# XuyangBai/D3Feat

Measured on AMD Instinct MI355X. Metric: fragments/sec (30k-pt clouds), higher is better.
Workload: dtype f32; 1 GPU; SURVEY §8d config #2: synthetic 3DMatch room fragment, 300k raw pts -> grid subsample 0.03 m (~29k pts per cloud) -> self-pair -> 5-level pyramid -> full KPFCNN forward (random-init weights (reference initialiser, seed 42), 14.1M params)...; points_per_cloud=29369, fragments_per_gpu=2141, parallelism=fragment-dp1, fragments_per_replay=12, engine_fallbacks=0, engine_isolated_replays=0

## Files before the change

### d3feat_amd/_lib.py

```python
import ctypes as C
import os

_HERE = os.path.dirname(os.path.abspath(__file__))
LIB_PATH = os.environ.get("D3FEAT_AMD_LIB") or os.path.join(_HERE, "lib", "libd3feat_amd.so")

D3F_OK = 0
ERRORS = {-1: "HIP runtime / kernel launch failure", -2: "workspace too small", -3: "invalid argument"}
ST_EMPTY_ELEMENT, ST_NEG_CELL, ST_KEY_RANGE, ST_HIT_OVERFLOW, ST_OUT_OVERFLOW, ST_KEY_WIDTH = 1, 2, 4, 8, 16, 32
PAD_NUM_SUPPORTS = -2147483648
NEIGHBOR_CAP = 1024
MAX_BATCH = 255
TOPK_MAX = 8192
PAIRS_KMAX = 1024

_vp, _sz, _i, _f = C.c_void_p, C.c_size_t, C.c_int, C.c_float

SIGNATURES = {
    "d3f_version": (_i, []),
    "d3f_trace_marker": (_i, [_i, _vp]),
    "d3f_pack_status": (_i, [_vp, _vp, _i, _vp, _i, _vp, _i, _vp, _i, _vp, _i, _i, _i, _vp]),
    "d3f_grid_subsample_workspace_bytes": (_sz, [_i, _i, _i, _i]),
    "d3f_batch_grid_subsample": (_i, [_vp, _i, _vp, _i, _f, _vp, _i, _vp, _i, _vp, _vp, _vp, _vp, _vp, _vp, _sz, _vp]),
    "d3f_batch_grid_subsample_async": (_i, [_vp, _i, _vp, _i, _f, _vp, _i, _i, _i, _vp, _vp, _vp, _sz, _vp]),
    "d3f_batch_grid_subsample_async_inplace": (_i, [_vp, _i, _vp, _i, _f, _vp, _i, _i, _vp, _vp, _vp, _sz, _vp]),
    "d3f_stack_self_pair": (_i, [_vp, _i, _vp, _i, _vp, _vp, _vp, _vp]),
    "d3f_radius_neighbors_workspace_bytes": (_sz, [_i, _i, _i]),
    "d3f_batch_radius_neighbors": (_i, [_vp, _i, _vp, _i, _vp, _vp, _i, _f, _vp, _i, _i, _i, _vp, _vp, _sz, _vp]),
    "d3f_neighbor_grid_bytes": (_sz, [_i, _i]),
    "d3f_neighbor_grid_order_offset": (_sz, [_i, _i]),
    "d3f_neighbor_grid_build": (_i, [_vp, _i, _vp, _i, _f, _vp, _sz, _vp]),
    "d3f_neighbor_grid_search": (_i, [_vp, _sz, _i, _vp, _i, _vp, _i, _f, _i, _vp, _i, _i, _i, _i, _i, _f, _i, _vp, _vp]),
    "d3f_neighbor_grid_search_ordered": (_i, [_vp, _sz, _i, _vp, _i, _vp, _i, _f, _vp, _sz, _vp, _i, _i, _i, _i, _i, _f, _i, _vp, _vp]),
    "d3f_neighbor_grid_inv_offset": (_sz, [_i, _i]),
    "d3f_neighbor_grid_xyz_offset": (_sz, [_i, _i]),
    "d3f_row_positive": (_i, [_vp, _i, _i, _i, _vp, _vp, _i, _vp]),
    "d3f_kpconv_aggregate": (_i, [_vp, _i, _vp, _i, _vp, _i, _i, _vp, _i, _i, _vp, _vp, _i, _f, _i, _i, _vp, _vp, _vp, _vp,
                                  _vp, _i, _vp]),
    "d3f_kpconv_fused_c1": (_i, [_vp, _i, _vp, _i, _vp, _i, _i, _vp, _i, _vp, _i, _f, _i, _i, _vp, _i, _vp, _vp, _vp, _i, _i,
                                 _f, _vp, _i, _vp, _vp, _vp, _i, _vp]),
    "d3f_kpconv_fused32": (_i, [_vp, _i, _vp, _i, _vp, _i, _i, _vp, _i, _vp, _vp, _i, _f, _i, _i, _vp, _vp, _vp, _vp, _i, _i, _f, _vp,
                                _i, _vp, _vp, _vp, _i, _vp]),
    "d3f_kpconv_fused_supported": (_i, [_i, _i, _i, _i, _i]),
    "d3f_kpconv_pack_weights": (_i, [_vp, _i, _i, _vp, _vp]),
    "d3f_kpconv_fused": (_i, [_vp, _i, _vp, _i, _vp, _i, _i, _vp, _i, _i, _vp, _vp, _i, _f, _i, _i, _vp, _i, _vp, _vp, _vp, _i, _i,
                              _f, _vp, _i, _vp, _vp, _vp, _i, _vp]),
    "d3f_kpconv_fused32_x3": (_i, [_vp, _i, _vp, _i, _vp, _i, _i, _vp, _i, _vp, _vp, _i, _f, _i, _i, _vp, _vp, _vp, _vp, _i, _i, _f, _vp,
                                   _i, _vp, _vp, _vp, _i, _vp]),
    "d3f_kpconv_packed_x3_bytes": (_sz, [_i, _i]),
    "d3f_kpconv_pack_weights_x3": (_i, [_vp, _i, _i, _vp, _vp]),
    "d3f_kpconv_fused_x3": (_i, [_vp, _i, _vp, _i, _vp, _i, _i, _vp, _i, _i, _vp, _vp, _i, _f, _i, _i, _vp, _i, _vp, _vp, _vp, _i, _i,
                                 _f, _vp, _i, _vp, _vp, _vp, _i, _vp]),
    "d3f_gemm_workspace_bytes": (_sz, [_i, _i, _i, _i]),
    "d3f_gemm_bf16_workspace_bytes": (_sz, [_i, _i, _i, _i]),
    "d3f_gemm_f32": (_i, [_vp, _i, _vp, _i, _vp, _i, _i, _i, _i, _vp, _vp, _vp, _vp, _i, _i, _f, _vp, _sz, _vp, _i, _vp]),
    "d3f_gemm_upsample_cat_f32": (_i, [_vp, _i, _i, _i, _vp, _i, _vp, _i, _i, _vp, _i, _vp, _i, _i, _i, _vp, _vp, _i, _f, _vp, _sz,
                                       _vp, _vp, _i, _vp]),
    "d3f_ind_max_pool": (_i, [_vp, _i, _i, _i, _vp, _i, _i, _i, _vp, _i, _vp, _vp, _vp, _vp, _i, _vp]),
    "d3f_closest_pool_cat": (_i, [_vp, _i, _i, _i, _vp, _i, _i, _vp, _i, _i, _vp, _i, _vp, _vp, _vp]),
    "d3f_affine_act": (_i, [_vp, _i, _i, _i, _vp, _vp, _vp, _i, _i, _f, _vp, _i, _vp, _vp]),
    "d3f_pack_descriptors": (_i, [_vp, _vp, _i, _i, _vp, _i, _vp, _i, _vp, _vp]),
    "d3f_pack_descriptors_to": (_i, [_vp, _vp, _i, _i, _vp, _i, _vp, _i, _vp, _vp, _i, _i, _i, _vp, _vp, _vp]),
    "d3f_topk_workspace_bytes": (_sz, [_i, _i, _i, _i]),
    "d3f_topk_records": (_i, [_vp, _i, _vp, _i, _i, _vp, _i, _i, _vp, _vp, _i, _i, _i, _vp, _i, _i, _vp, _i, _vp, _vp, _vp, _vp, _sz,
                              _vp]),
    "d3f_feature_nn_workspace_bytes": (_sz, [_i]),
    "d3f_feature_nn": (_i, [_vp, _i, _i, _vp, _i, _i, _i, _vp, _vp, _vp, _sz, _vp]),
    "d3f_mutual_matches_workspace_bytes": (_sz, [_i]),
    "d3f_mutual_matches": (_i, [_vp, _i, _vp, _i, _vp, _vp, _vp, _sz, _vp]),
    "d3f_ransac_hypotheses": (_i, [_vp, _i, _vp, _i, _vp, _i, _f, _f, C.c_uint64, C.c_uint64, _i, _vp, _vp, _vp]),
    "d3f_ransac_draw": (_i, [C.c_uint64, C.c_uint64, _i, _i]),
    "d3f_neighbor_grid_score": (_i, [_vp, _sz, _i, _vp, _i, _vp, _i, _f, _vp, _vp, _vp, _vp]),
    "d3f_register_pairs_workspace_bytes": (_sz, [_i, _i, _i, _i]),
    "d3f_register_pairs": (_i, [_vp, _i, _i, _i, _i, _vp, _vp, _i, _i, _f, _i, _f, _f, _i, _i, C.c_uint64, _vp, _f] + [_vp] * 11
                           + [_sz, _vp]),
# ... 45 lines not shown
```

### d3feat_amd/csrc/grid_subsample.hip

```cpp
#include <cstdlib>
#include "prims.h"
#include "radix_sort.h"

#define GS_EMPTY 0xFFFFFFFFFFFFFFFFull
#define GS_KEYBITS 56
#define GS_KEYMASK ((1ull << GS_KEYBITS) - 1ull)
#define GS_MAX_PROBE 4096

__constant__ unsigned long long D3F_CHAIN_DEV[D3F_NCHAIN] = {
    13ull, 29ull, 59ull, 127ull, 257ull, 541ull, 1109ull, 2357ull, 5087ull, 10273ull, 20753ull, 42043ull, 85229ull,
    172933ull, 351061ull, 712697ull, 1447153ull, 2938679ull, 5967347ull, 12117689ull, 24607243ull, 49969847ull,
    101473717ull, 206062531ull, 418451333ull, 849749479ull, 1725587117ull, 3504151727ull};

struct GsElem {
    float org[3];
    int pad0;
    unsigned long long NX, NY, NZ;
    long long bbase;
};

static unsigned long long gs_chain_ge(long long n) {
    for (int j = 0; j < D3F_NCHAIN; ++j)
        if ((long long)D3F_CHAIN_HOST[j] >= n) return D3F_CHAIN_HOST[j];
    return D3F_CHAIN_HOST[D3F_NCHAIN - 1];
// ... 11 lines not shown
}
__device__ __forceinline__ void gs_prep(const unsigned* __restrict__ bbox, const int* __restrict__ offs, int B, float dl,
                                        GsElem* __restrict__ el, int* __restrict__ status, RsMeta* __restrict__ smeta,
                                        int n_cap) {
    __shared__ unsigned long long sCells[256];
    const int b = threadIdx.x;
    unsigned long long cells = 0ull;
    if (b < B) {
        GsElem e;
        e.pad0 = 0;
        const int len = offs[b + 1] - offs[b];
        if (len <= 0) {
            atomicOr(&status[1], D3F_ST_EMPTY_ELEMENT);
            e.org[0] = e.org[1] = e.org[2] = 0.f;
            e.NX = e.NY = e.NZ = 1;
        } else {
            const float inv = __fdiv_rn(1.0f, dl);
            float mx[3];
#pragma unroll
            for (int d = 0; d < 3; ++d) {
                float mn = d3f_ord2f(__hip_atomic_load(&bbox[b * 6 + d], __ATOMIC_RELAXED, __HIP_MEMORY_SCOPE_AGENT));
                mx[d] = d3f_ord2f(__hip_atomic_load(&bbox[b * 6 + 3 + d], __ATOMIC_RELAXED, __HIP_MEMORY_SCOPE_AGENT));
                e.org[d] = __fmul_rn(floorf(__fmul_rn(mn, inv)), dl);
            }
            e.NX = (unsigned long long)fmaxf(floorf(__fdiv_rn(__fsub_rn(mx[0], e.org[0]), dl)), 0.f) + 1ull;
            e.NY = (unsigned long long)fmaxf(floorf(__fdiv_rn(__fsub_rn(mx[1], e.org[1]), dl)), 0.f) + 1ull;
            e.NZ = (unsigned long long)fmaxf(floorf(__fdiv_rn(__fsub_rn(mx[2], e.org[2]), dl)), 0.f) + 1ull;
        }
        long long base = 0;
        for (int j = 0; j < b; ++j) {
            long long l = offs[j + 1] - offs[j];
            unsigned long long nb = D3F_CHAIN_DEV[D3F_NCHAIN - 1];
            for (int c = 0; c < D3F_NCHAIN; ++c)
                if ((long long)D3F_CHAIN_DEV[c] >= l) { nb = D3F_CHAIN_DEV[c]; break; }
            base += (long long)nb;
        }
        e.bbase = base;
        el[b] = e;
        const double c = (double)e.NX * (double)e.NY * (double)e.NZ;
        cells = c >= 1.8e19 ? 0xFFFFFFFFFFFFFFFFull : e.NX * e.NY * e.NZ;
    }
    if (!smeta) return;
    sCells[threadIdx.x] = cells;
    __syncthreads();
    if (threadIdx.x == 0) {
        unsigned long long mx = 1ull;
        for (int j = 0; j < B; ++j) mx = sCells[j] > mx ? sCells[j] : mx;
        int kb = gs_bits(mx - 1ull);
        if (kb < 1) kb = 1;
        const int eb = gs_bits((unsigned long long)(B - 1));
        RsMeta m;
        m.n = min(offs[B], n_cap);
        m.kb = kb;
        m.bits = kb + eb;
        if (m.bits > 32) {
            atomicOr(&status[1], D3F_ST_KEY_WIDTH);
            m.n = 0;
            m.bits = 8;
        }
        m.npass = (m.bits + 7) / 8;
        *smeta = m;
    }
}
struct GsPrepEpi {
    const unsigned* bbox; const int* offs; int B; float dl; GsElem* el; int* status; RsMeta* smeta; int n_cap;
    __device__ __forceinline__ void operator()() const { gs_prep(bbox, offs, B, dl, el, status, smeta, n_cap); }
};

__global__ void __launch_bounds__(256) gs_insert_kernel(const float* __restrict__ pts, int N, const int* __restrict__ offs,
                                                        int B, float dl, const GsElem* __restrict__ el,
                                                        unsigned long long* __restrict__ tkey, unsigned* __restrict__ tfirst,
                                                        unsigned long long capmask, int* __restrict__ slot,
                                                        int* __restrict__ status) {
    const int i = blockIdx.x * blockDim.x + threadIdx.x;
    if (i >= min(N, offs[B])) return;
    const int b = d3f_find_elem(offs, B, i);
    const GsElem e = el[b];
    const float fx = floorf(__fdiv_rn(__fsub_rn(pts[3 * (size_t)i + 0], e.org[0]), dl));
    const float fy = floorf(__fdiv_rn(__fsub_rn(pts[3 * (size_t)i + 1], e.org[1]), dl));
    const float fz = floorf(__fdiv_rn(__fsub_rn(pts[3 * (size_t)i + 2], e.org[2]), dl));
    int st = 0;
    if (fx < 0.f || fy < 0.f || fz < 0.f) st |= D3F_ST_NEG_CELL;
    const unsigned long long ix = (unsigned long long)fmaxf(fx, 0.f), iy = (unsigned long long)fmaxf(fy, 0.f),
                             iz = (unsigned long long)fmaxf(fz, 0.f);
    const unsigned long long key = ix + e.NX * iy + e.NX * e.NY * iz;
    if (key > GS_KEYMASK) st |= D3F_ST_KEY_RANGE;
    if (st) atomicOr(&status[1], st);
    const unsigned long long word = ((unsigned long long)b << GS_KEYBITS) | (key & GS_KEYMASK);
    unsigned long long h = gs_mix(word) & capmask;
    bool placed = false;
    for (int probe = 0; probe < GS_MAX_PROBE; ++probe) {
        unsigned long long prev = atomicCAS(&tkey[h], GS_EMPTY, word);
        if (prev == GS_EMPTY || prev == word) { placed = true; break; }
        h = (h + 1) & capmask;
    }
    if (!placed) atomicOr(&status[1], D3F_ST_OUT_OVERFLOW);
    atomicMin(&tfirst[h], (unsigned)i);
    slot[i] = (int)h;
}

struct GsMarkIn {
    const int* n_dev; const int* slot; const unsigned* tfirst;
    __device__ __forceinline__ int operator()(int i) const { return (i < *n_dev && tfirst[slot[i]] == (unsigned)i) ? 1 : 0; }
};

__global__ void __launch_bounds__(256) gs_chain_kernel(int N, const int* __restrict__ slot, const unsigned* __restrict__ tfirst,
                                                       const unsigned long long* __restrict__ tkey,
                                                       const int* __restrict__ vscan, const int* __restrict__ vbase,
                                                       int* __restrict__ pvid,
                                                       unsigned long long* __restrict__ vkey, int* __restrict__ vhead,
                                                       int* __restrict__ vcnt, int* __restrict__ pnext,
                                                       const int* __restrict__ n_dev) {
    const int i = blockIdx.x * blockDim.x + threadIdx.x;
// ... 291 lines not shown
        int run = wbase + x - s;
#pragma unroll
        for (int k = 0; k < 4; ++k) {
            const int u = tile * GS_TILE + tid * 4 + k;
            if (u < hi) A.cd[o + hi - 1 - u] = run;
            run += c[k];
        }
        if (tid == 0) A.tsum[o / GS_TILE + b + tile] = tot;
    }
    if (!d3f_last_block(counter + b, (unsigned)((hi + GS_TILE - 1) / GS_TILE))) return;
    gs_order_scan_sums(A, j, b, wsum);
}

__global__ void __launch_bounds__(256) gs_order_place_kernel(GsOrderArgs A, int j) {
    const int b = blockIdx.y;
    int M, lo, hi, nb;
    bool last;
    if (!gs_round(A, b, j, M, lo, hi, nb, last)) return;
    const int t = blockIdx.x * 256 + threadIdx.x;
    const int o = A.offs[b];
    const long long bbase = A.el[b].bbase;
    const bool next = !last && j + 1 < D3F_NCHAIN;
    const int nbn = next ? (int)D3F_CHAIN_DEV[j + 1] : 1;
    int id = -1, pos = -1;
    if (t < hi) {
        id = (t < lo) ? A.P[j & 1][o + t] : t;
        const int bk = A.bkt[j & 1][o + t];
        int r = 0;
        for (int q = A.bh[j & 1][bbase + bk]; q >= 0; q = A.nx[j & 1][o + q]) r += (q > t) ? 1 : 0;
        const int f = A.bf[j & 1][bbase + bk];
        const int dest = A.cd[o + f] + A.tsum[o / GS_TILE + b + (hi - 1 - f) / GS_TILE] + r;
        A.P[(j + 1) & 1][o + dest] = id;
        if (last) A.vpos[A.moffs[b] + id] = dest;
        pos = dest;
    } else if (next && t < min(M, nbn)) {
        id = pos = t;
    }
    if (next && id >= 0) {
        const int bk = gs_mod(A.vkey[A.moffs[b] + id], (unsigned)nbn, 1.0 / (double)nbn);
        atomicMin(&A.bf[(j + 1) & 1][bbase + bk], pos);
        atomicAdd(&A.bc[(j + 1) & 1][bbase + bk], 1);
        A.nx[(j + 1) & 1][o + pos] = atomicExch(&A.bh[(j + 1) & 1][bbase + bk], pos);
        A.bkt[(j + 1) & 1][o + pos] = bk;
    }
}

#include "gs_small.h"

__global__ void __launch_bounds__(RS_THREADS) gs_sortkey_kernel(const float* __restrict__ pts, const float* const* __restrict__ ptrs,
                                                                const int* __restrict__ offs, int B,
                                                                float dl, const GsElem* __restrict__ el,
                                                                const RsMeta* __restrict__ smeta, unsigned* __restrict__ skey,
                                                                unsigned* __restrict__ hist, int* __restrict__ status) {
    __shared__ unsigned sHist[256];
    __shared__ int sOffs[D3F_MAX_BATCH + 1];
    __shared__ GsElem sEl[D3F_MAX_BATCH];
    __shared__ const float* sBase[D3F_MAX_BATCH];
    const int n = smeta->n, kb = smeta->kb;
    const int tile = blockIdx.x;
    if ((long long)tile * RS_TILE >= (long long)n) return;
    for (int t = threadIdx.x; t <= B; t += RS_THREADS) sOffs[t] = offs[t];
    for (int t = threadIdx.x; t < B; t += RS_THREADS) {
        sEl[t] = el[t];
        sBase[t] = ptrs ? ptrs[t] - 3 * (size_t)offs[t] : pts;
    }
    __syncthreads();
    const int w = threadIdx.x >> 6, lane = threadIdx.x & 63;
    const int base = tile * RS_TILE + w * RS_WAVE_ITEMS + lane;
    const int wlo = tile * RS_TILE + w * RS_WAVE_ITEMS, whi = min(wlo + RS_WAVE_ITEMS, n) - 1;
    int b0 = 0;
    while (b0 + 1 < B && wlo >= sOffs[b0 + 1]) ++b0;
    const bool one_cloud = (b0 + 1 >= B) || whi < sOffs[b0 + 1];
    unsigned key[RS_ROUNDS], vm = 0u;
    int st = 0;
#pragma unroll
    for (int r = 0; r < RS_ROUNDS; ++r) {
        const int i = base + r * 64;
        key[r] = 0u;
        if (i < n) {
            int b = b0;
            if (!one_cloud)
                while (b + 1 < B && i >= sOffs[b + 1]) ++b;
            const float ox = sEl[b].org[0], oy = sEl[b].org[1], oz = sEl[b].org[2];
            const unsigned NX = (unsigned)sEl[b].NX, NY = (unsigned)sEl[b].NY;
            const float* __restrict__ P = sBase[b];
            const float fx = floorf(__fdiv_rn(__fsub_rn(P[3 * (size_t)i + 0], ox), dl));
            const float fy = floorf(__fdiv_rn(__fsub_rn(P[3 * (size_t)i + 1], oy), dl));
            const float fz = floorf(__fdiv_rn(__fsub_rn(P[3 * (size_t)i + 2], oz), dl));
            if (fx < 0.f || fy < 0.f || fz < 0.f) st |= D3F_ST_NEG_CELL;
            const unsigned ix = (unsigned)fmaxf(fx, 0.f), iy = (unsigned)fmaxf(fy, 0.f), iz = (unsigned)fmaxf(fz, 0.f);
            const unsigned k = ix + NX * (iy + NY * iz);
            key[r] = (kb < 32 ? ((unsigned)b << kb) : 0u) | (kb < 32 ? (k & ((1u << kb) - 1u)) : k);
            skey[i] = key[r];
            vm |= 1u << r;
        }
    }
    if (st) atomicOr(&status[1], st);
    rs_tile_histogram(key, vm, 0, sHist, hist + (size_t)tile * 256);
}

__global__ void __launch_bounds__(256) gs_heads_kernel(int N, const RsMeta* __restrict__ smeta, const unsigned* __restrict__ key0,
                                                       const unsigned* __restrict__ key1, const unsigned* __restrict__ val0,
                                                       const unsigned* __restrict__ val1, unsigned* __restrict__ fbits) {
    const int j = blockIdx.x * blockDim.x + threadIdx.x;
    if (j >= min(N, smeta->n)) return;
    const unsigned* __restrict__ ks = (smeta->npass & 1) ? key1 : key0;
    const unsigned* __restrict__ vs = (smeta->npass & 1) ? val1 : val0;
    const unsigned k = ks[j];
    if (j == 0 || ks[j - 1] != k) {
        const unsigned i = vs[j];
        atomicOr(&fbits[i >> 5], 1u << (i & 31u));
    }
}
struct GsBitsIn {
    const unsigned* fbits;
    __device__ __forceinline__ int operator()(int w) const { return __popc(fbits[w]); }
};
__global__ void __launch_bounds__(256) gs_runs_kernel(int N, const RsMeta* __restrict__ smeta, const unsigned* __restrict__ key0,
                                                      const unsigned* __restrict__ key1, const unsigned* __restrict__ val0,
                                                      const unsigned* __restrict__ val1, GsRankBits rank,
                                                      const float* __restrict__ pts, const float* const* __restrict__ ptrs,
                                                      const int* __restrict__ offs, unsigned long long* __restrict__ vkey,
                                                      float* __restrict__ bary) {
    __shared__ float sx[256], sy[256], sz[256];
    __shared__ unsigned sk[256];
    const int n = min(N, smeta->n);
    const int j0 = blockIdx.x * 256;
    if (j0 >= n) return;
    const int t = threadIdx.x, j = j0 + t;
    const unsigned* __restrict__ ks = (smeta->npass & 1) ? key1 : key0;
    const unsigned* __restrict__ vs = (smeta->npass & 1) ? val1 : val0;
    unsigned k = 0u, pi = 0u, kprev = 0u;
    float px = 0.f, py = 0.f, pz = 0.f;
    if (j < n) {
        k = ks[j];
        pi = vs[j];
        kprev = j > 0 ? ks[j - 1] : 0u;
        if (ptrs) {
            const int b = smeta->kb < 32 ? (int)(k >> smeta->kb) : 0;
            pts = ptrs[b] - 3 * (size_t)offs[b];
        }
        px = pts[3 * (size_t)pi + 0]; py = pts[3 * (size_t)pi + 1]; pz = pts[3 * (size_t)pi + 2];
    }
    sx[t] = px; sy[t] = py; sz[t] = pz;
    sk[t] = k;
    __syncthreads();
    if (j >= n || (j != 0 && kprev == k)) return;
    const int v = rank((int)pi);
    float ax = px, ay = py, az = pz;
    int c = 1;
    const int lim = min(256, n - j0);
// ... 48 lines not shown
    const int n = vcnt[v], st = sbase ? d3f_scan_at(vstart, sbase, v) : vstart[v];
    const size_t dest = (size_t)moffs[b] + (size_t)vpos[v];
    if (dest >= (size_t)out_cap) {
        atomicOr(&status[1], D3F_ST_OUT_OVERFLOW);
        return;
    }
    float sx = 0.f, sy = 0.f, sz = 0.f;
    for (int t = 0; t < n; ++t) {
        const size_t i = (size_t)sorted[st + t];
        sx = __fadd_rn(sx, pts[3 * i + 0]);
        sy = __fadd_rn(sy, pts[3 * i + 1]);
        sz = __fadd_rn(sz, pts[3 * i + 2]);
    }
    const float sc = (float)(1.0 / (double)n);
    out_p[3 * dest + 0] = __fmul_rn(sx, sc);
    out_p[3 * dest + 1] = __fmul_rn(sy, sc);
    out_p[3 * dest + 2] = __fmul_rn(sz, sc);
    if (fdim > 0) {
        const float cf = (float)n;
        for (int f = 0; f < fdim; ++f) {
            float s = 0.f;
            for (int t = 0; t < n; ++t) s = __fadd_rn(s, feat[(size_t)sorted[st + t] * fdim + f]);
            out_f[dest * fdim + f] = __fdiv_rn(s, cf);
        }
    }
}

__global__ void __launch_bounds__(256) gs_fill_kernel(int* __restrict__ p, size_t n, int v) {
    const size_t i = (size_t)blockIdx.x * blockDim.x + threadIdx.x;
    if (i < n) p[i] = v;
}
__global__ void __launch_bounds__(256) gs_labels_kernel(int N, int ldim, const int* __restrict__ cls,
                                                        const int* __restrict__ pvid, const int* __restrict__ moffs, int B,
                                                        const int* __restrict__ vpos, int* __restrict__ out_c) {
    const int i = blockIdx.x * blockDim.x + threadIdx.x;
    if (i >= N) return;
    const int v = pvid[i];
    const int b = d3f_find_elem(moffs, B, v);
    const size_t dest = (size_t)moffs[b] + (size_t)vpos[v];
    for (int l = 0; l < ldim; ++l) atomicMax(&out_c[dest * ldim + l], cls[(size_t)i * ldim + l]);
}

struct GsLayout {
    size_t cap;
    long long bucket_total;
};
static GsLayout gs_layout(int N, int B, int keys = -1) {
    GsLayout L;
    L.cap = 64;
    const size_t nk = (size_t)((keys > 0 && keys < N) ? keys : (N > 0 ? N : 1));
    while (L.cap < (size_t)2 * nk) L.cap <<= 1;
    L.bucket_total = (long long)(2.24 * (double)N) + 16ll * B + 64;
    return L;
}

extern "C" size_t d3f_grid_subsample_workspace_bytes(int N, int B, int fdim, int ldim) {
    (void)fdim; (void)ldim;
    if (N < 0 || B < 1) return 0;
    GsLayout L = gs_layout(N, B);
    size_t n = (size_t)(N > 0 ? N : 1);
    size_t bytes = 0;
    bytes += d3f_align((B + 1) * sizeof(int)) * 2 + d3f_align((B + 2) * sizeof(int));
    bytes += d3f_align(B * 6 * sizeof(unsigned));
    bytes += d3f_align(B * sizeof(GsElem));
    bytes += d3f_align(L.cap * sizeof(unsigned long long));
    bytes += d3f_align(L.cap * sizeof(int));
    bytes += d3f_align(n * sizeof(unsigned long long));
    bytes += 16 * d3f_align(n * sizeof(int));
    bytes += 6 * d3f_align((size_t)L.bucket_total * sizeof(int));
    bytes += d3f_align((n / GS_TILE + B + 8) * sizeof(int));
    bytes += 2 * d3f_align(d3f_scan_base_ints(N) * sizeof(int)) + d3f_align((4 + D3F_NCHAIN * (size_t)B) * sizeof(unsigned));
    bytes += d3f_align(rs_hist_words(N) * sizeof(unsigned)) + d3f_align((n / 32 + 2) * sizeof(unsigned)) +
             d3f_align(3 * n * sizeof(float)) + d3f_align(sizeof(RsMeta));
    bytes += d3f_align(7 * (size_t)B * (n < 16384 ? n : 16384) * sizeof(float)) + 256 + 2 * d3f_align(B * sizeof(int));
    return bytes + 4096;
}

template <int T, int R>
static int gs_small_launch(const GsSmallArgs& A, float* sub_points, int* sub_lens_dev, int* status_dev, hipStream_t stream) {
    static std::atomic<unsigned long long> lds_done{0ull};
    const void* const fns[] = {(const void*)gs_small_kernel<T, R>};
    if (d3f_opt_in_lds(lds_done, fns, (int)gss_lds_bytes<T, R>(GSS_NB_MAX)) != D3F_OK) return D3F_ERR_HIP;
    gs_small_kernel<T, R><<<A.B, T, gss_lds_bytes<T, R>(A.nbmax), stream>>>(A);
    D3F_LAUNCH_CHECK();
    gs_small_pack_kernel<<<d3f_cdiv(A.out_cap, 256), 256, 0, stream>>>(A, sub_points, sub_lens_dev, status_dev);
    D3F_LAUNCH_CHECK();
    return D3F_OK;
}
static int gs_run_small(const float* points, int N, const int* lens_dev, int B, float dl, float* sub_points, int M_cap, int elem_cap,
                        int pc, int* sub_lens_dev, int* status_dev, void* workspace, size_t workspace_bytes, hipStream_t stream) {
    if (elem_cap <= 0 || elem_cap > M_cap) elem_cap = M_cap;
    if (elem_cap > pc) elem_cap = pc;
    D3fArena ar(workspace, workspace_bytes);
    GsSmallArgs A;
    A.stage = ar.take<float>(3 * (size_t)B * (size_t)elem_cap);
    A.recs = ar.take<float>(4 * (size_t)B * (size_t)elem_cap);
    A.mcount = ar.take<int>(B);
    A.cflags = ar.take<int>(B);
    if (!ar.ok) return D3F_ERR_WORKSPACE;
    A.pts = points; A.lens = lens_dev; A.B = B; A.dl = dl; A.elem_cap = elem_cap; A.out_cap = M_cap;
    A.nbmax = GSS_NB_MAX;
    for (int j = 0; j < D3F_NCHAIN; ++j)
        if ((long long)D3F_CHAIN_HOST[j] >= (long long)elem_cap) { A.nbmax = (int)D3F_CHAIN_HOST[j]; break; }
    if (A.nbmax > GSS_NB_MAX) A.nbmax = GSS_NB_MAX;
    if (A.nbmax < 1109) A.nbmax = 1109;
    if (pc <= 2048) return gs_small_launch<256, 8>(A, sub_points, sub_lens_dev, status_dev, stream);
// ... 224 lines not shown
```

### d3feat_amd/csrc/radix_sort.h

```cpp
#pragma once
#include "common.h"

#define RS_THREADS 512
#define RS_WAVES (RS_THREADS / 64)
#define RS_ROUNDS 16
#define RS_TILE (RS_THREADS * RS_ROUNDS)
#define RS_WAVE_ITEMS (64 * RS_ROUNDS)
#define RS_MAX_PASSES 4

struct RsMeta {
    int n;
    int bits;
    int npass;
    int kb;
};

#define RS_SCATTER_LDS_BYTES ((2 * RS_WAVES * 256 + 256 + 16 + 2 * RS_TILE) * 4)
static inline int rs_tiles(int n_cap) { return d3f_cdiv(n_cap > 0 ? n_cap : 1, RS_TILE); }
static inline size_t rs_hist_words(int n_cap) { return (size_t)rs_tiles(n_cap) * 256; }

#ifdef __HIPCC__
__device__ __forceinline__ void rs_tile_histogram(const unsigned (&key)[RS_ROUNDS], unsigned valid_mask, int shift,
                                                  unsigned* __restrict__ sHist, unsigned* __restrict__ hist_row) {
    if (threadIdx.x < 256) sHist[threadIdx.x] = 0u;
    __syncthreads();
#pragma unroll
    for (int r = 0; r < RS_ROUNDS; ++r)
        if (valid_mask & (1u << r)) atomicAdd(&sHist[(key[r] >> shift) & 255u], 1u);
    __syncthreads();
    if (threadIdx.x < 256) hist_row[threadIdx.x] = sHist[threadIdx.x];
}

__global__ void __launch_bounds__(RS_THREADS) rs_hist_kernel(const RsMeta* __restrict__ meta, int pass,
                                                             const unsigned* __restrict__ key0,
                                                             const unsigned* __restrict__ key1,
                                                             unsigned* __restrict__ hist) {
    __shared__ unsigned sHist[256];
    const int n = meta->n;
    if (pass >= meta->npass) return;
    const int tile = blockIdx.x;
    if ((long long)tile * RS_TILE >= (long long)n) return;
    const unsigned* __restrict__ src = (pass & 1) ? key1 : key0;
    const int w = threadIdx.x >> 6, lane = threadIdx.x & 63;
    const int base = tile * RS_TILE + w * RS_WAVE_ITEMS + lane;
    unsigned key[RS_ROUNDS], vm = 0u;
#pragma unroll
    for (int r = 0; r < RS_ROUNDS; ++r) {
        const int pos = base + r * 64;
        key[r] = 0u;
        if (pos < n) { key[r] = src[pos]; vm |= 1u << r; }
    }
    rs_tile_histogram(key, vm, pass * 8, sHist, hist + (size_t)tile * 256);
}

__global__ void __launch_bounds__(RS_THREADS) rs_scatter_kernel(const RsMeta* __restrict__ meta, int pass,
                                                                unsigned* __restrict__ key0, unsigned* __restrict__ key1,
                                                                unsigned* __restrict__ val0, unsigned* __restrict__ val1,
                                                                const unsigned* __restrict__ hist) {
    extern __shared__ __attribute__((aligned(16))) unsigned rs_lds[];
    unsigned (*sCnt)[256] = (unsigned (*)[256])rs_lds;
    unsigned (*sPart)[256] = (unsigned (*)[256])(rs_lds + RS_WAVES * 256);
    unsigned* sBase = rs_lds + 2 * RS_WAVES * 256;
    unsigned* sScan = sBase + 256;
    unsigned* sKey = sScan + 16;
    unsigned* sVal = sKey + RS_TILE;
    const int n = meta->n;
    if (pass >= meta->npass) return;
    const int tile = blockIdx.x;
    if ((long long)tile * RS_TILE >= (long long)n) return;
    const int live = (n + RS_TILE - 1) / RS_TILE;
    const unsigned* __restrict__ ksrc = (pass & 1) ? key1 : key0;
    const unsigned* __restrict__ vsrc = (pass & 1) ? val1 : val0;
    unsigned* __restrict__ kdst = (pass & 1) ? key0 : key1;
    unsigned* __restrict__ vdst = (pass & 1) ? val0 : val1;
    const int tid = threadIdx.x, w = tid >> 6, lane = tid & 63;
    const int shift = pass * 8;

    const int base = tile * RS_TILE + w * RS_WAVE_ITEMS + lane;
    unsigned key[RS_ROUNDS], val[RS_ROUNDS];
#pragma unroll
    for (int r = 0; r < RS_ROUNDS; ++r) {
        const int pos = base + r * 64;
        key[r] = 0u;
        val[r] = (unsigned)pos;
        if (pos < n) {
            key[r] = ksrc[pos];
            if (pass > 0) val[r] = vsrc[pos];
        }
    }
    {
        uint4 bef = make_uint4(0u, 0u, 0u, 0u), tot = make_uint4(0u, 0u, 0u, 0u);
        const uint4* __restrict__ rows = (const uint4*)hist + lane;
        int t = w;
        for (; t + 7 * RS_WAVES < live; t += 8 * RS_WAVES) {
            uint4 v[8];
#pragma unroll
            for (int u = 0; u < 8; ++u) v[u] = rows[(size_t)(t + u * RS_WAVES) * 64];
#pragma unroll
            for (int u = 0; u < 8; ++u) {
                tot.x += v[u].x; tot.y += v[u].y; tot.z += v[u].z; tot.w += v[u].w;
                if (t + u * RS_WAVES < tile) { bef.x += v[u].x; bef.y += v[u].y; bef.z += v[u].z; bef.w += v[u].w; }
            }
        }
        for (; t < live; t += RS_WAVES) {
            const uint4 v = rows[(size_t)t * 64];
            tot.x += v.x; tot.y += v.y; tot.z += v.z; tot.w += v.w;
            if (t < tile) { bef.x += v.x; bef.y += v.y; bef.z += v.z; bef.w += v.w; }
        }
        ((uint4*)sCnt[w])[lane] = tot;
        ((uint4*)sPart[w])[lane] = bef;
    }
    __syncthreads();
    {
        unsigned total = 0u, before = 0u;
        if (tid < 256) {
#pragma unroll
            for (int q = 0; q < RS_WAVES; ++q) { total += sCnt[q][tid]; before += sPart[q][tid]; }
        }
        unsigned x = total;
#pragma unroll
        for (int d = 1; d < 64; d <<= 1) {
            const unsigned y = (unsigned)__shfl_up((int)x, d, 64);
            if (lane >= d) x += y;
        }
        if (lane == 63) sScan[w] = x;
        __syncthreads();
#pragma unroll
        for (int q = 0; q < RS_WAVES; ++q)
            if (tid < 256) sCnt[q][tid] = 0u;
        unsigned wb = 0u;
#pragma unroll
        for (int q = 0; q < 4; ++q) wb += (q < w) ? sScan[q] : 0u;
        if (tid < 256) sBase[tid] = wb + x - total + before;
        __syncthreads();
    }
    unsigned rank[RS_ROUNDS];
    volatile unsigned* myCnt = sCnt[w];
#pragma unroll
    for (int r = 0; r < RS_ROUNDS; ++r) {
        const bool valid = (base + r * 64) < n;
        const unsigned dg = (key[r] >> shift) & 255u;
        unsigned long long peers = __ballot(valid);
#pragma unroll
        for (int bit = 0; bit < 8; ++bit) {
            const bool one = (dg >> bit) & 1u;
            const unsigned long long m = __ballot(one);
            peers &= one ? m : ~m;
        }
        rank[r] = 0u;
        if (valid) {
            const unsigned prev = myCnt[dg];
            const unsigned below = (unsigned)__popcll(peers & d3f_lanemask_lt());
            rank[r] = prev + below;
            __builtin_amdgcn_wave_barrier();
            if (below == 0u) myCnt[dg] = prev + (unsigned)__popcll(peers);
        }
        __builtin_amdgcn_wave_barrier();
    }
    __syncthreads();
    {
        unsigned cnt = 0u;
        if (tid < 256) {
#pragma unroll
            for (int q = 0; q < RS_WAVES; ++q) cnt += sCnt[q][tid];
        }
        unsigned x = cnt;
#pragma unroll
        for (int d = 1; d < 64; d <<= 1) {
            const unsigned y = (unsigned)__shfl_up((int)x, d, 64);
            if (lane >= d) x += y;
        }
        if (lane == 63) sScan[w] = x;
        __syncthreads();
        if (tid < 256) {
            unsigned wb = 0u;
#pragma unroll
            for (int q = 0; q < 4; ++q) wb += (q < w) ? sScan[q] : 0u;
            const unsigned loc = wb + x - cnt;
            unsigned run = loc;
#pragma unroll
            for (int q = 0; q < RS_WAVES; ++q) {
                const unsigned c = sCnt[q][tid];
                sCnt[q][tid] = run;
                run += c;
            }
            sBase[tid] -= loc;
        }
    }
    __syncthreads();
#pragma unroll
    for (int r = 0; r < RS_ROUNDS; ++r) {
        if ((base + r * 64) < n) {
            const unsigned dg = (key[r] >> shift) & 255u;
            const unsigned pl = myCnt[dg] + rank[r];
            sKey[pl] = key[r];
            sVal[pl] = val[r];
        }
    }
    __syncthreads();
    const int tile_n = min(RS_TILE, n - tile * RS_TILE);
#pragma unroll
    for (int r = 0; r < RS_ROUNDS; ++r) {
        const int pl = r * RS_THREADS + tid;
        if (pl < tile_n) {
            const unsigned k = sKey[pl];
            const unsigned dest = sBase[(k >> shift) & 255u] + (unsigned)pl;
            kdst[dest] = k;
            vdst[dest] = sVal[pl];
        }
    }
}
#endif

static inline int rs_sort_launch(const RsMeta* meta, int n_cap, unsigned* key0, unsigned* key1, unsigned* val0, unsigned* val1,
                                 unsigned* hist, hipStream_t stream) {
    const int tiles = rs_tiles(n_cap);
    static std::atomic<unsigned long long> lds_done{0ull};
    const void* const fns[] = {(const void*)rs_scatter_kernel};
    if (d3f_opt_in_lds(lds_done, fns, RS_SCATTER_LDS_BYTES) != D3F_OK) return D3F_ERR_HIP;
    for (int p = 0; p < RS_MAX_PASSES; ++p) {
        if (p > 0) {
            rs_hist_kernel<<<tiles, RS_THREADS, 0, stream>>>(meta, p, key0, key1, hist);
            D3F_LAUNCH_CHECK();
        }
        rs_scatter_kernel<<<tiles, RS_THREADS, RS_SCATTER_LDS_BYTES, stream>>>(meta, p, key0, key1, val0, val1, hist);
        D3F_LAUNCH_CHECK();
    }
    return D3F_OK;
}
```

### include/d3feat_amd.h

```cpp
#ifndef D3FEAT_AMD_H
#define D3FEAT_AMD_H

#include <stddef.h>
#include <stdint.h>

#ifdef __cplusplus
extern "C" {
#endif

#define D3F_OK 0
#define D3F_ERR_HIP (-1)
#define D3F_ERR_WORKSPACE (-2)
#define D3F_ERR_ARG (-3)

#define D3F_ST_EMPTY_ELEMENT 1
#define D3F_ST_NEG_CELL 2
#define D3F_ST_KEY_RANGE 4
#define D3F_ST_HIT_OVERFLOW 8
#define D3F_ST_OUT_OVERFLOW 16
#define D3F_ST_KEY_WIDTH 32

#define D3F_NB_NO_KMAX 2
#define D3F_PAD_NUM_SUPPORTS (-2147483647 - 1)

#define D3F_MAX_BATCH 255
#define D3F_NEIGHBOR_CAP 1024
#define D3F_TOPK_MAX 8192
#define D3F_PAIRS_KMAX 1024
#define D3F_NUM_KP_MAX 16

int d3f_version(void);

int d3f_trace_marker(int id, void* stream);
int d3f_pack_status(int* dst, const int* a, int na, const int* b, int nb, const int* c, int nc, const int* d, int nd,
                    int* clear, int nclear, int clear_first, int clear_step, void* stream);


size_t d3f_grid_subsample_workspace_bytes(int N, int B, int fdim, int ldim);
int d3f_batch_grid_subsample_async(const float* points, int N_cap, const int* lens_dev, int B, float dl,
                                   float* sub_points, int M_cap, int elem_cap, int elem_points_cap, int* sub_lens_dev,
                                   int* status_dev, void* workspace, size_t workspace_bytes, void* stream);
int d3f_batch_grid_subsample_async_inplace(const float* const* clouds_dev, int N_cap, const int* lens_dev, int B, float dl,
                                           float* sub_points, int M_cap, int elem_cap, int* sub_lens_dev, int* status_dev,
                                           void* workspace, size_t workspace_bytes, void* stream);

int d3f_stack_self_pair(const float* pts, int M_cap, const int* lens_in_dev, int B, float* out, int* lens_out_dev,
                        int* total_dev, void* stream);
int d3f_batch_grid_subsample(const float* points, int N, const int* lens_dev, int B, float dl,
                             const float* features, int fdim, const int* classes, int ldim,
                             float* sub_points, float* sub_features, int* sub_classes, int* sub_lens_dev,
                             int* status_host, void* workspace, size_t workspace_bytes, void* stream);

size_t d3f_radius_neighbors_workspace_bytes(int Nq, int Ns, int B);
int d3f_batch_radius_neighbors(const float* queries, int Nq, const float* supports, int Ns,
                               const int* q_lens_dev, const int* s_lens_dev, int B, float radius,
                               int* out, int ld, int width, int pad_value, int* status_dev,
                               void* workspace, size_t workspace_bytes, void* stream);

size_t d3f_neighbor_grid_bytes(int Ns, int B);
size_t d3f_neighbor_grid_order_offset(int Ns, int B);
int d3f_neighbor_grid_build(const float* supports, int Ns, const int* s_lens_dev, int B, float radius,
                            void* grid, size_t grid_bytes, void* stream);
int d3f_neighbor_grid_search(const void* grid, size_t grid_bytes, int Ns, const float* queries, int Nq,
                             const int* q_lens_dev, int B, float radius, int queries_are_supports,
                             int* out, int ld, int width, int pad_value, int cap, int first_only, float nn_hint,
                             int reset_status, int* status_dev, void* stream);
#define D3F_NB_INTERNAL 4
int d3f_neighbor_grid_search_ordered(const void* grid, size_t grid_bytes, int Ns, const float* queries, int Nq,
                                     const int* q_lens_dev, int B, float radius, const void* query_grid, size_t query_grid_bytes,
                                     int* out, int ld, int width, int pad_value, int cap, int first_only, float nn_hint, int flags,
                                     int* status_dev, void* stream);
size_t d3f_neighbor_grid_inv_offset(int Ns, int B);
size_t d3f_neighbor_grid_xyz_offset(int Ns, int B);



int d3f_row_positive(const void* f, int Ns, int ldf, int Cin, unsigned char* row_pos, const int* Ns_dev, int feat_bf16,
                     void* stream);
int d3f_kpconv_aggregate(const float* q, int Nq, const float* s, int Ns, const int* idx, int ld_idx, int K,
                         const void* f, int ldf, int Cin, const unsigned char* row_pos, const float* kp_host,
                         int num_kp, float KP_extent, int influence, int aggregation, float* wf, float* inv_cnt,
                         const int* Nq_dev, const int* Ns_dev, const int* q_order, int feat_bf16, void* stream);

int d3f_kpconv_fused_c1(const float* q, int Nq, const float* s, int Ns, const int* idx, int ld_idx, int K,
                        const float* f, int ldf, const float* kp_host, int num_kp, float KP_extent, int influence,
                        int aggregation, const float* W, int Cout, const float* col_scale, const float* col_shift,
                        const float* residual, int ldr, int leaky, float alpha, void* out, int ldo,
                        const int* Nq_dev, const int* Ns_dev, const int* q_order, int out_bf16, void* stream);

int d3f_kpconv_fused32(const float* q, int Nq, const float* s, int Ns, const int* idx, int ld_idx, int K,
                       const void* f, int ldf, const unsigned char* row_pos, const float* kp_host, int num_kp,
// ... 121 lines not shown
```

Before: 1862 fragments/s.

## Use variable-width radix digits and sort only cell-key bits in grid subsample

Result: no change. 1877 fragments/s, median of 6 (+0.8%).

```diff
diff --git a/d3feat_amd/_lib.py b/d3feat_amd/_lib.py
--- a/d3feat_amd/_lib.py
+++ b/d3feat_amd/_lib.py
@@ -20,6 +20,7 @@
     "d3f_trace_marker": (_i, [_i, _vp]),
     "d3f_pack_status": (_i, [_vp, _vp, _i, _vp, _i, _vp, _i, _vp, _i, _vp, _i, _i, _i, _vp]),
     "d3f_grid_subsample_workspace_bytes": (_sz, [_i, _i, _i, _i]),
+    "d3f_radix_sort_plan": (_i, [_i, _vp, _vp]),
     "d3f_batch_grid_subsample": (_i, [_vp, _i, _vp, _i, _f, _vp, _i, _vp, _i, _vp, _vp, _vp, _vp, _vp, _vp, _sz, _vp]),
     "d3f_batch_grid_subsample_async": (_i, [_vp, _i, _vp, _i, _f, _vp, _i, _i, _i, _vp, _vp, _vp, _sz, _vp]),
     "d3f_batch_grid_subsample_async_inplace": (_i, [_vp, _i, _vp, _i, _f, _vp, _i, _i, _vp, _vp, _vp, _sz, _vp]),
diff --git a/d3feat_amd/csrc/grid_subsample.hip b/d3feat_amd/csrc/grid_subsample.hip
--- a/d3feat_amd/csrc/grid_subsample.hip
+++ b/d3feat_amd/csrc/grid_subsample.hip
@@ -87,13 +87,13 @@
         RsMeta m;
         m.n = min(offs[B], n_cap);
         m.kb = kb;
-        m.bits = kb + eb;
-        if (m.bits > 32) {
+        m.bits = kb;
+        if (kb + eb > 32) {
             atomicOr(&status[1], D3F_ST_KEY_WIDTH);
             m.n = 0;
             m.bits = 8;
         }
-        m.npass = (m.bits + 7) / 8;
+        rs_plan(m.bits, &m.d, &m.npass);
         *smeta = m;
     }
 }
@@ -491,7 +491,7 @@
                                                                 float dl, const GsElem* __restrict__ el,
                                                                 const RsMeta* __restrict__ smeta, unsigned* __restrict__ skey,
                                                                 unsigned* __restrict__ hist, int* __restrict__ status) {
-    __shared__ unsigned sHist[256];
+    __shared__ unsigned sHist[RS_BINS];
     __shared__ int sOffs[D3F_MAX_BATCH + 1];
     __shared__ GsElem sEl[D3F_MAX_BATCH];
     __shared__ const float* sBase[D3F_MAX_BATCH];
@@ -535,7 +535,8 @@
         }
     }
     if (st) atomicOr(&status[1], st);
-    rs_tile_histogram(key, vm, 0, sHist, hist + (size_t)tile * 256);
+    const RsDigit dig(smeta, 0);
+    rs_tile_histogram(key, vm, dig, sHist, hist + (size_t)tile * dig.nb);
 }
 
 __global__ void __launch_bounds__(256) gs_heads_kernel(int N, const RsMeta* __restrict__ smeta, const unsigned* __restrict__ key0,
@@ -690,6 +691,12 @@
     while (L.cap < (size_t)2 * nk) L.cap <<= 1;
     L.bucket_total = (long long)(2.24 * (double)N) + 16ll * B + 64;
     return L;
+}
+
+extern "C" int d3f_radix_sort_plan(int bits, int* digit_bits, int* passes) {
+    if (bits < 1 || bits > 32 || !digit_bits || !passes) return D3F_ERR_ARG;
+    rs_plan(bits, digit_bits, passes);
+    return D3F_OK;
 }
 
 extern "C" size_t d3f_grid_subsample_workspace_bytes(int N, int B, int fdim, int ldim) {
diff --git a/d3feat_amd/csrc/radix_sort.h b/d3feat_amd/csrc/radix_sort.h
--- a/d3feat_amd/csrc/radix_sort.h
+++ b/d3feat_amd/csrc/radix_sort.h
@@ -7,39 +7,68 @@
 #define RS_TILE (RS_THREADS * RS_ROUNDS)
 #define RS_WAVE_ITEMS (64 * RS_ROUNDS)
 #define RS_MAX_PASSES 4
+#ifndef RS_DMAX
+#define RS_DMAX 9
+#endif
+#define RS_BINS (1 << RS_DMAX)
+#define RS_DPT (RS_BINS / RS_THREADS)
+static_assert(RS_DMAX >= 9 && RS_DMAX <= 10, "RS_THREADS threads scan RS_BINS digits, the column partials alias the tile");
 
 struct RsMeta {
     int n;
     int bits;
     int npass;
     int kb;
+    int d;
 };
 
-#define RS_SCATTER_LDS_BYTES ((2 * RS_WAVES * 256 + 256 + 16 + 2 * RS_TILE) * 4)
+static inline __host__ __device__ void rs_plan(int bits, int* d, int* npass) {
+    const int np = (bits + RS_DMAX - 1) / RS_DMAX;
+    int w = (bits + np - 1) / np;
+    if (w < 8) w = 8;
+    *d = w;
+    *npass = (bits + w - 1) / w;
+}
+
+#define RS_SCATTER_LDS_BYTES ((RS_WAVES * RS_BINS + RS_BINS + 16 + 2 * RS_TILE) * 4)
 static inline int rs_tiles(int n_cap) { return d3f_cdiv(n_cap > 0 ? n_cap : 1, RS_TILE); }
-static inline size_t rs_hist_words(int n_cap) { return (size_t)rs_tiles(n_cap) * 256; }
+static inline size_t rs_hist_words(int n_cap) { return (size_t)rs_tiles(n_cap) * RS_BINS; }
 
 #ifdef __HIPCC__
-__device__ __forceinline__ void rs_tile_histogram(const unsigned (&key)[RS_ROUNDS], unsigned valid_mask, int shift,
+struct RsDigit {
+    int shift, nb;
+    unsigned mask;
+    __device__ __forceinline__ RsDigit(const RsMeta* __restrict__ meta, int pass) {
+        const int d = meta->d, bits = meta->bits;
+        shift = pass * d;
+        nb = 1 << d;
+        const unsigned keymask = bits >= 32 ? 0xFFFFFFFFu : ((1u << bits) - 1u);
+        mask = (keymask >> shift) & (unsigned)(nb - 1);
+    }
+    __device__ __forceinline__ unsigned operator()(unsigned key) const { return (key >> shift) & mask; }
+};
+
+__device__ __forceinline__ void rs_tile_histogram(const unsigned (&key)[RS_ROUNDS], unsigned valid_mask, const RsDigit dig,
                                                   unsigned* __restrict__ sHist, unsigned* __restrict__ hist_row) {
-    if (threadIdx.x < 256) sHist[threadIdx.x] = 0u;
+    for (int t = threadIdx.x; t < dig.nb; t += RS_THREADS) sHist[t] = 0u;
     __syncthreads();
 #pragma unroll
     for (int r = 0; r < RS_ROUNDS; ++r)
-        if (valid_mask & (1u << r)) atomicAdd(&sHist[(key[r] >> shift) & 255u], 1u);
-    __syncthreads();
-    if (threadIdx.x < 256) hist_row[threadIdx.x] = sHist[threadIdx.x];
+        if (valid_mask & (1u << r)) atomicAdd(&sHist[dig(key[r])], 1u);
+    __syncthreads();
+    for (int t = threadIdx.x; t < dig.nb; t += RS_THREADS) hist_row[t] = sHist[t];
 }
 
 __global__ void __launch_bounds__(RS_THREADS) rs_hist_kernel(const RsMeta* __restrict__ meta, int pass,
                                                              const unsigned* __restrict__ key0,
                                                              const unsigned* __restrict__ key1,
                                                              unsigned* __restrict__ hist) {
-    __shared__ unsigned sHist[256];
+    __shared__ unsigned sHist[RS_BINS];
     const int n = meta->n;
     if (pass >= meta->npass) return;
     const int tile = blockIdx.x;
     if ((long long)tile * RS_TILE >= (long long)n) return;
+    const RsDigit dig(meta, pass);
     const unsigned* __restrict__ src = (pass & 1) ? key1 : key0;
     const int w = threadIdx.x >> 6, lane = threadIdx.x & 63;
     const int base = tile * RS_TILE + w * RS_WAVE_ITEMS + lane;
@@ -50,7 +79,7 @@
         key[r] = 0u;
         if (pos < n) { key[r] = src[pos]; vm |= 1u << r; }
     }
-    rs_tile_histogram(key, vm, pass * 8, sHist, hist + (size_t)tile * 256);
+    rs_tile_histogram(key, vm, dig, sHist, hist + (size_t)tile * dig.nb);
 }
 
 __global__ void __launch_bounds__(RS_THREADS) rs_scatter_kernel(const RsMeta* __restrict__ meta, int pass,
@@ -58,12 +87,12 @@
                                                                 unsigned* __restrict__ val0, unsigned* __restrict__ val1,
                                                                 const unsigned* __restrict__ hist) {
     extern __shared__ __attribute__((aligned(16))) unsigned rs_lds[];
-    unsigned (*sCnt)[256] = (unsigned (*)[256])rs_lds;
-    unsigned (*sPart)[256] = (unsigned (*)[256])(rs_lds + RS_WAVES * 256);
-    unsigned* sBase = rs_lds + 2 * RS_WAVES * 256;
-    unsigned* sScan = sBase + 256;
+    unsigned (*sCnt)[RS_BINS] = (unsigned (*)[RS_BINS])rs_lds;
+    unsigned* sBase = rs_lds + RS_WAVES * RS_BINS;
+    unsigned* sScan = sBase + RS_BINS;
     unsigned* sKey = sScan + 16;
     unsigned* sVal = sKey + RS_TILE;
+    unsigned (*sPart)[RS_BINS] = (unsigned (*)[RS_BINS])sKey;
     const int n = meta->n;
     if (pass >= meta->npass) return;
     const int tile = blockIdx.x;
@@ -74,7 +103,8 @@
     unsigned* __restrict__ kdst = (pass & 1) ? key0 : key1;
     unsigned* __restrict__ vdst = (pass & 1) ? val0 : val1;
     const int tid = threadIdx.x, w = tid >> 6, lane = tid & 63;
-    const int shift = pass * 8;
+    const RsDigit dig(meta, pass);
+    const int d = meta->d, nb = dig.nb;
 
     const int base = tile * RS_TILE + w * RS_WAVE_ITEMS + lane;
     unsigned key[RS_ROUNDS], val[RS_ROUNDS];
@@ -88,14 +118,15 @@
             if (pass > 0) val[r] = vsrc[pos];
         }
     }
-    {
+    for (int c = 0; c < (nb >> 8); ++c) {
         uint4 bef = make_uint4(0u, 0u, 0u, 0u), tot = make_uint4(0u, 0u, 0u, 0u);
-        const uint4* __restrict__ rows = (const uint4*)hist + lane;
+        const uint4* __restrict__ rows = (const uint4*)(hist + c * 256) + lane;
+        const size_t rs4 = (size_t)(nb >> 2);
         int t = w;
         for (; t + 7 * RS_WAVES < live; t += 8 * RS_WAVES) {
             uint4 v[8];
 #pragma unroll
-            for (int u = 0; u < 8; ++u) v[u] = rows[(size_t)(t + u * RS_WAVES) * 64];
+            for (int u = 0; u < 8; ++u) v[u] = rows[(size_t)(t + u * RS_WAVES) * rs4];
 #pragma unroll
             for (int u = 0; u < 8; ++u) {
                 tot.x += v[u].x; tot.y += v[u].y; tot.z += v[u].z; tot.w += v[u].w;
@@ -103,35 +134,46 @@
             }
         }
         for (; t < live; t += RS_WAVES) {
-            const uint4 v = rows[(size_t)t * 64];
+            const uint4 v = rows[(size_t)t * rs4];
             tot.x += v.x; tot.y += v.y; tot.z += v.z; tot.w += v.w;
             if (t < tile) { bef.x += v.x; bef.y += v.y; bef.z += v.z; bef.w += v.w; }
         }
-        ((uint4*)sCnt[w])[lane] = tot;
-        ((uint4*)sPart[w])[lane] = bef;
+        ((uint4*)(sCnt[w] + c * 256))[lane] = tot;
+        ((uint4*)(sPart[w] + c * 256))[lane] = bef;
     }
     __syncthreads();
     {
-        unsigned total = 0u, before = 0u;
-        if (tid < 256) {
-#pragma unroll
-            for (int q = 0; q < RS_WAVES; ++q) { total += sCnt[q][tid]; before += sPart[q][tid]; }
-        }
-        unsigned x = total;
-#pragma unroll
-        for (int d = 1; d < 64; d <<= 1) {
-            const unsigned y = (unsigned)__shfl_up((int)x, d, 64);
-            if (lane >= d) x += y;
+        unsigned total[RS_DPT], before[RS_DPT], x = 0u;
+#pragma unroll
+        for (int i = 0; i < RS_DPT; ++i) {
+            const int dg = tid * RS_DPT + i;
+            total[i] = before[i] = 0u;
+            if (dg < nb) {
+#pragma unroll
+                for (int q = 0; q < RS_WAVES; ++q) { total[i] += sCnt[q][dg]; before[i] += sPart[q][dg]; }
+            }
+            x += total[i];
+        }
+        const unsigned mine = x;
+#pragma unroll
+        for (int s = 1; s < 64; s <<= 1) {
+            const unsigned y = (unsigned)__shfl_up((int)x, s, 64);
+            if (lane >= s) x += y;
         }
         if (lane == 63) sScan[w] = x;
         __syncthreads();
 #pragma unroll
-        for (int q = 0; q < RS_WAVES; ++q)
-            if (tid < 256) sCnt[q][tid] = 0u;
-        unsigned wb = 0u;
-#pragma unroll
-        for (int q = 0; q < 4; ++q) wb += (q < w) ? sScan[q] : 0u;
-        if (tid < 256) sBase[tid] = wb + x - total + before;
+        for (int i = 0; i < RS_DPT; ++i)
+#pragma unroll
+            for (int q = 0; q < RS_WAVES; ++q) sCnt[q][tid * RS_DPT + i] = 0u;
+        unsigned run = x - mine;
+#pragma unroll
+        for (int q = 0; q < RS_WAVES; ++q) run += (q < w) ? sScan[q] : 0u;
+#pragma unroll
+        for (int i = 0; i < RS_DPT; ++i) {
+            sBase[tid * RS_DPT + i] = run + before[i];
+            run += total[i];
+        }
         __syncthreads();
     }
     unsigned rank[RS_ROUNDS];
@@ -139,13 +181,15 @@
 #pragma unroll
     for (int r = 0; r < RS_ROUNDS; ++r) {
         const bool valid = (base + r * 64) < n;
-        const unsigned dg = (key[r] >> shift) & 255u;
+        const unsigned dg = dig(key[r]);
         unsigned long long peers = __ballot(valid);
 #pragma unroll
-        for (int bit = 0; bit < 8; ++bit) {
-            const bool one = (dg >> bit) & 1u;
-            const unsigned long long m = __ballot(one);
-            peers &= one ? m : ~m;
+        for (int bit = 0; bit < RS_DMAX; ++bit) {
+            if (bit < 8 || bit < d) {
+                const bool one = (dg >> bit) & 1u;
+                const unsigned long long m = __ballot(one);
+                peers &= one ? m : ~m;
+            }
         }
         rank[r] = 0u;
         if (valid) {
@@ -159,40 +203,44 @@
     }
     __syncthreads();
     {
-        unsigned cnt = 0u;
-        if (tid < 256) {
-#pragma unroll
-            for (int q = 0; q < RS_WAVES; ++q) cnt += sCnt[q][tid];
-        }
-        unsigned x = cnt;
-#pragma unroll
-        for (int d = 1; d < 64; d <<= 1) {
-            const unsigned y = (unsigned)__shfl_up((int)x, d, 64);
-            if (lane >= d) x += y;
+        unsigned cnt[RS_DPT], x = 0u;
+#pragma unroll
+        for (int i = 0; i < RS_DPT; ++i) {
+            cnt[i] = 0u;
+#pragma unroll
+            for (int q = 0; q < RS_WAVES; ++q) cnt[i] += sCnt[q][tid * RS_DPT + i];
+            x += cnt[i];
+        }
+        const unsigned mine = x;
+#pragma unroll
+        for (int s = 1; s < 64; s <<= 1) {
+            const unsigned y = (unsigned)__shfl_up((int)x, s, 64);
+            if (lane >= s) x += y;
         }
         if (lane == 63) sScan[w] = x;
         __syncthreads();
-        if (tid < 256) {
-            unsigned wb = 0u;
-#pragma unroll
-            for (int q = 0; q < 4; ++q) wb += (q < w) ? sScan[q] : 0u;
-            const unsigned loc = wb + x - cnt;
+        unsigned loc = x - mine;
+#pragma unroll
+        for (int q = 0; q < RS_WAVES; ++q) loc += (q < w) ? sScan[q] : 0u;
+#pragma unroll
+        for (int i = 0; i < RS_DPT; ++i) {
+            const int dg = tid * RS_DPT + i;
             unsigned run = loc;
 #pragma unroll
             for (int q = 0; q < RS_WAVES; ++q) {
-                const unsigned c = sCnt[q][tid];
-                sCnt[q][tid] = run;
+                const unsigned c = sCnt[q][dg];
+                sCnt[q][dg] = run;
                 run += c;
             }
-            sBase[tid] -= loc;
+            sBase[dg] -= loc;
+            loc += cnt[i];
         }
     }
     __syncthreads();
 #pragma unroll
     for (int r = 0; r < RS_ROUNDS; ++r) {
         if ((base + r * 64) < n) {
-            const unsigned dg = (key[r] >> shift) & 255u;
-            const unsigned pl = myCnt[dg] + rank[r];
+            const unsigned pl = myCnt[dig(key[r])] + rank[r];
             sKey[pl] = key[r];
             sVal[pl] = val[r];
         }
@@ -204,7 +252,7 @@
         const int pl = r * RS_THREADS + tid;
         if (pl < tile_n) {
             const unsigned k = sKey[pl];
-            const unsigned dest = sBase[(k >> shift) & 255u] + (unsigned)pl;
+            const unsigned dest = sBase[dig(k)] + (unsigned)pl;
             kdst[dest] = k;
             vdst[dest] = sVal[pl];
         }
diff --git a/include/d3feat_amd.h b/include/d3feat_amd.h
--- a/include/d3feat_amd.h
+++ b/include/d3feat_amd.h
@@ -37,6 +37,7 @@
 
 
 size_t d3f_grid_subsample_workspace_bytes(int N, int B, int fdim, int ldim);
+int d3f_radix_sort_plan(int bits, int* digit_bits, int* passes);
 int d3f_batch_grid_subsample_async(const float* points, int N_cap, const int* lens_dev, int B, float dl,
                                    float* sub_points, int M_cap, int elem_cap, int elem_points_cap, int* sub_lens_dev,
                                    int* status_dev, void* workspace, size_t workspace_bytes, void* stream);
```
